# InternRobotics/InternNav

Measured on NVIDIA H100. Metric: InternVLA-N1 policy-steps/sec (batch RGB-D+text->action), higher is better.
Workload: dtype bf16

## Files before the change

### include/n1b200.h

```cpp
#ifndef N1B200_H_
#define N1B200_H_

#include <stddef.h>
#include <stdint.h>

#ifdef __cplusplus
extern "C" {
#endif

typedef struct n1_ctx* n1_handle;

enum {
  N1_OK = 0,
  N1_ERR_UNKNOWN = -1,
  N1_ERR_ARG = -2,
  N1_ERR_CUDA = -3,
  N1_ERR_NO_DEVICE = -4,
  N1_ERR_TMA = -5,
  N1_ERR_WEIGHT = -6,
  N1_ERR_WORKSPACE = -7
};

enum { N1_F32 = 0, N1_BF16 = 1 };

// ... 182 lines not shown
                int accumulate, void* ws, size_t ws_bytes, void* stream);
int n1_op_scale_cols(const void* x_bf16, int ld_x, const void* gamma_f32, const void* add_bf16_or_null, int ld_add,
                     void* out_bf16, int ld_out, int64_t rows, int cols, void* stream);
int n1_op_patchify_depth(const void* img_f32, void* out_bf16, int n_img, int ldk, void* stream);
int n1_op_adamw(void* master_f32, void* working_bf16_or_null, const void* grad_f32, void* m_f32, void* v_f32, int64_t n,
                float lr, float beta1, float beta2, float eps, float weight_decay, int step, void* stream);

void n1_prof_enable(int on);
void n1_prof_add(int64_t gemm_launches, int64_t total_launches);
int n1_prof_read(double* gemm_ms, double* gemm_flops, int64_t* gemm_launches, int64_t* total_launches);
int n1_prof_read_shapes(int32_t* mnk, int64_t* count, double* ms, int cap);

int n1_op_gemm(const void* A_bf16, int lda, const void* W_bf16, int ldw, void* out, int ldo, int M, int N, int K,
               const float* bias, const float* gamma, const void* residual_bf16, int ldr, int act, int out_fp32,
               void* stream);
int n1_op_ff_block(const void* x_bf16, int ldx, const float* ln_w, const float* ln_b, float eps, const void* w1_bf16,
                   const float* b1, const void* w2_bf16, const float* b2, void* out_bf16, int ldo, int M, void* stream);
int n1_op_dec_sa_block(void* x_bf16, int ldx, const float* ln_w, const float* ln_b, float eps, const void* w_qkv_bf16,
                       const float* b_qkv, const void* w_o_bf16, const float* b_o, int B, int Ns, int T, int causal,
                       void* stream);
int n1_op_dec_ca_block(void* x_bf16, int ldx, const float* ln_w, const float* ln_b, float eps, const void* w_q_bf16,
                       const float* b_q, const void* w_o_bf16, const float* b_o, const void* kv_bf16, int ldkv, int mtok,
                       int B, int Ns, int T, void* stream);
int n1_op_layernorm(const void* x_bf16, int ldx, void* y_bf16, int ldy, const float* w, const float* b, int rows, int D,
                    float eps, int rms, void* stream);
int n1_op_mod_norm(const void* x_bf16, int ldx, const float* w, const void* mod_bf16, int ld_mod, int rows_per_group,
                   const void* res_bf16, int ldr, void* out_bf16, int ldo, int64_t rows, int D, float eps, int mode,
                   void* stream);
int n1_op_add(const void* a_bf16, const void* b_bf16, void* out_bf16, int64_t n, void* stream);
int n1_op_action_embed(const float* lat, const float* w, const float* b, const float* pos, void* out_bf16, int64_t rows,
                       int T, int D, void* stream);
int n1_op_cfg_euler(const void* pred_bf16, int ld, int64_t n, int cfg, float scale, float dt, float* lat, void* stream);
int n1_op_attention(const void* q, const void* k, const void* v, void* o, int ldq, int ldk, int ldv, int ldo, int heads_q,
                    int heads_kv, int head_dim, int batch, int seq_q, int seq_k, const int32_t* cu_q,
                    const int32_t* cu_k, int max_seq_q, int kv_div, int causal, float scale, void* stream);

int n1_op_attention_ex(const void* q, const void* k, const void* v, void* o, int ldq, int ldk, int ldv, int ldo, int heads_q,
                       int heads_kv, int head_dim, int batch, const int32_t* cu_seqlens, int max_seq, int64_t total_rows,
                       int causal, float scale, int* used_tcgen05, void* stream);

int n1_op_attention_cache(const void* q, int ldq, int64_t q_rows, const void* k, const void* v, int ldkv, int64_t kv_rows,
                          void* o, int ldo, const int32_t* cu_q, const int32_t* ctx, const int32_t* row0, int batch,
                          int max_chunk, int heads_q, int heads_kv, float scale, void* stream);

#ifdef __cplusplus
}
// ... 3 lines not shown
```

### internnav_b200/_lib.py

```python
import ctypes
import os
import threading

import torch

_HERE = os.path.dirname(os.path.abspath(__file__))
LIB_PATH = os.path.join(_HERE, "libn1b200.so")

_lib = None
_lock = threading.Lock()

c_void_p, c_int, c_size_t, c_float, c_char_p = (
    ctypes.c_void_p, ctypes.c_int, ctypes.c_size_t, ctypes.c_float, ctypes.c_char_p)


class N1Error(RuntimeError):
    def __init__(self, code, msg):
        super().__init__("n1b200 error %d: %s" % (code, msg))
        self.code = code


class TensorDesc(ctypes.Structure):
    _fields_ = [("name", c_char_p), ("data", c_void_p), ("dtype", ctypes.c_int32), ("ndim", ctypes.c_int32),
                ("shape", ctypes.c_int64 * 4)]
# ... 18 lines not shown
    "n1_navdp_eps": (c_int, [c_void_p, c_void_p, c_size_t, c_void_p, c_void_p, c_int, c_void_p, c_void_p, c_void_p,
                             c_int, c_int, c_int, c_void_p]),
    "n1_navdp_sample": (c_int, [c_void_p, c_void_p, c_size_t, c_void_p, c_void_p, c_void_p, c_void_p, c_void_p,
                                c_int, c_int, c_int, c_int, c_void_p]),
    "n1_ddpm_tables": (c_int, [c_int, ctypes.POINTER(c_float)]),
    "n1_rgb_tokens_workspace_bytes": (c_size_t, [c_void_p, c_int]),
    "n1_rgb_tokens": (c_int, [c_void_p, c_void_p, c_size_t, c_void_p, c_void_p, c_int, c_void_p]),
    "n1_traj_to_actions": (c_int, [c_void_p, c_int, c_int, c_int, ctypes.c_double, ctypes.c_double, c_int, c_int, c_int,
                                   c_void_p, c_void_p, c_void_p, c_void_p]),
    "n1_prof_enable": (None, [c_int]),
    "n1_prof_add": (None, [ctypes.c_int64, ctypes.c_int64]),
    "n1_prof_read": (c_int, [ctypes.POINTER(ctypes.c_double), ctypes.POINTER(ctypes.c_double),
                             ctypes.POINTER(ctypes.c_int64), ctypes.POINTER(ctypes.c_int64)]),
    "n1_prof_read_shapes": (c_int, [ctypes.POINTER(ctypes.c_int32), ctypes.POINTER(ctypes.c_int64),
                                    ctypes.POINTER(ctypes.c_double), c_int]),
    "n1_op_gemm": (c_int, [c_void_p, c_int, c_void_p, c_int, c_void_p, c_int, c_int, c_int, c_int, c_void_p, c_void_p,
                           c_void_p, c_int, c_int, c_int, c_void_p]),
    "n1_op_ff_block": (c_int, [c_void_p, c_int, c_void_p, c_void_p, c_float, c_void_p, c_void_p, c_void_p, c_void_p, c_void_p,
                               c_int, c_int, c_void_p]),
    "n1_op_dec_sa_block": (c_int, [c_void_p, c_int, c_void_p, c_void_p, c_float, c_void_p, c_void_p, c_void_p, c_void_p,
                                   c_int, c_int, c_int, c_int, c_void_p]),
    "n1_op_dec_ca_block": (c_int, [c_void_p, c_int, c_void_p, c_void_p, c_float, c_void_p, c_void_p, c_void_p, c_void_p,
                                   c_void_p, c_int, c_int, c_int, c_int, c_int, c_void_p]),
    "n1_op_layernorm": (c_int, [c_void_p, c_int, c_void_p, c_int, c_void_p, c_void_p, c_int, c_int, c_float, c_int,
                                c_void_p]),
    "n1_op_mod_norm": (c_int, [c_void_p, c_int, c_void_p, c_void_p, c_int, c_int, c_void_p, c_int, c_void_p, c_int,
                               ctypes.c_int64, c_int, c_float, c_int, c_void_p]),
    "n1_op_add": (c_int, [c_void_p, c_void_p, c_void_p, ctypes.c_int64, c_void_p]),
    "n1_op_action_embed": (c_int, [c_void_p, c_void_p, c_void_p, c_void_p, c_void_p, ctypes.c_int64, c_int, c_int, c_void_p]),
    "n1_op_cfg_euler": (c_int, [c_void_p, c_int, ctypes.c_int64, c_int, c_float, c_float, c_void_p, c_void_p]),
    "n1_op_attention_ex": (c_int, [c_void_p, c_void_p, c_void_p, c_void_p, c_int, c_int, c_int, c_int, c_int, c_int, c_int,
                                   c_int, c_void_p, c_int, ctypes.c_int64, c_int, c_float, ctypes.POINTER(c_int), c_void_p]),
    "n1_op_attention": (c_int, [c_void_p, c_void_p, c_void_p, c_void_p, c_int, c_int, c_int, c_int, c_int, c_int, c_int,
                                c_int, c_int, c_int, c_void_p, c_void_p, c_int, c_int, c_int, c_float, c_void_p]),
    "n1_op_attention_cache": (c_int, [c_void_p, c_int, ctypes.c_int64, c_void_p, c_void_p, c_int, ctypes.c_int64, c_void_p,
                                      c_int, c_void_p, c_void_p, c_void_p, c_int, c_int, c_int, c_int, c_float, c_void_p]),
}

OP_RGBD, OP_GOAL, OP_DENOISE = 1, 2, 3
ACT_NONE, ACT_GELU, ACT_RELU, ACT_SWIGLU, ACT_GELU_TANH, ACT_SILU = 0, 1, 2, 3, 4, 5


def lib():
    global _lib
    with _lock:
        if _lib is None:
# ... 155 lines not shown
    if scale is None:
        scale = head_dim ** -0.5
    used = c_int(0)
    check(lib().n1_op_attention_ex(c_void_p(q.data_ptr()), c_void_p(k.data_ptr()), c_void_p(v.data_ptr()), ptr(o),
                                   q.stride(0), k.stride(0), v.stride(0), o.stride(0), heads_q, heads_kv, head_dim,
                                   cu_seqlens.numel() - 1, ptr(cu_seqlens), int(max_seq), q.shape[0], 1 if causal else 0,
                                   float(scale), ctypes.byref(used), stream_ptr()))
    return o, bool(used.value)


def attention_cache(q, k, v, heads_q, heads_kv, cu_q, ctx, row0, max_chunk, scale=None, out=None):
    assert q.dtype == k.dtype == v.dtype == torch.bfloat16 and q.stride(1) == 1 and k.stride(1) == 1 and v.stride(1) == 1
    assert k.stride(0) == v.stride(0) and k.shape[0] == v.shape[0]
    for t in (cu_q, ctx, row0):
        assert t.dtype == torch.int32 and t.is_cuda and t.is_contiguous()
    o = torch.empty(q.shape[0], heads_q * 128, device=q.device, dtype=torch.bfloat16) if out is None else out
    check(lib().n1_op_attention_cache(c_void_p(q.data_ptr()), q.stride(0), q.shape[0], c_void_p(k.data_ptr()),
                                      c_void_p(v.data_ptr()), k.stride(0), k.shape[0], ptr(o), o.stride(0), ptr(cu_q),
                                      ptr(ctx), ptr(row0), cu_q.numel() - 1, int(max_chunk), heads_q, heads_kv,
                                      float(128 ** -0.5 if scale is None else scale), stream_ptr()))
    return o


def ff_block(x, ln_w, ln_b, w1, b1, w2, b2, eps=1e-5, out=None):
    assert x.dtype == torch.bfloat16 and x.shape[1] == 384 and w1.shape == (1536, 384) and w2.shape == (384, 1536)
    assert w1.is_contiguous() and w2.is_contiguous() and x.stride(1) == 1
    if out is None:
        out = torch.empty(x.shape[0], 384, device=x.device, dtype=torch.bfloat16)
    check(lib().n1_op_ff_block(c_void_p(x.data_ptr()), x.stride(0), ptr(ln_w), ptr(ln_b), eps, ptr(w1), ptr(b1), ptr(w2),
                               ptr(b2), c_void_p(out.data_ptr()), out.stride(0), x.shape[0], stream_ptr()))
    return out


def dec_sa_block(x, ln_w, ln_b, w_qkv, b_qkv, w_o, b_o, B, Ns, T, causal=True, eps=1e-5):
    assert x.dtype == torch.bfloat16 and x.shape == (B * Ns * T, 384) and x.stride(1) == 1
    assert w_qkv.shape == (1152, 384) and w_o.shape == (384, 384)
    check(lib().n1_op_dec_sa_block(c_void_p(x.data_ptr()), x.stride(0), ptr(ln_w), ptr(ln_b), float(eps), ptr(w_qkv),
                                   ptr(b_qkv), ptr(w_o), ptr(b_o), B, Ns, T, 1 if causal else 0, stream_ptr()))
    return x


def dec_ca_block(x, ln_w, ln_b, w_q, b_q, w_o, b_o, kv, mtok, B, Ns, T, eps=1e-5):
    assert x.dtype == torch.bfloat16 and x.shape == (B * Ns * T, 384) and x.stride(1) == 1
    assert w_q.shape == (384, 384) and w_o.shape == (384, 384) and kv.shape[0] == B * mtok and kv.stride(1) == 1
    check(lib().n1_op_dec_ca_block(c_void_p(x.data_ptr()), x.stride(0), ptr(ln_w), ptr(ln_b), float(eps), ptr(w_q), ptr(b_q),
                                   ptr(w_o), ptr(b_o), c_void_p(kv.data_ptr()), kv.stride(0), mtok, B, Ns, T, stream_ptr()))
    return x
```

### internnav_b200/csrc/api.cu

```cuda
#include <string.h>

#include <string>
#include <vector>

#include "../../include/n1b200.h"
#include "n1_ops.h"
#include "resize.h"
#include "bwd_kernels.h"
#include "s1_model.h"
#include "s2_kernels.h"
#include "s2_model.h"
#include "weights.h"

using namespace n1;

struct n1_ctx {
  int device = 0;
  S1Model s1;
  S2Model s2;
};
struct n1_vit_plan_s {
  VitPlan* p;
};
struct n1_llm_plan_s {
// ... 735 lines not shown
    e.bias = bias, e.gamma = gamma, e.residual = B16(residual), e.ldr = ldr, e.act = act, e.out_fp32 = out_fp32;
    gemm_bf16(B16(A), lda, B16(W), ldw, out, ldo, M, N, K, e, S(stream));
  });
}

int n1_test_gemm(const void* A, int lda, const void* W, int ldw, void* out, int ldo, int M, int N, int K, const float* bias,
                 const float* gamma, const void* residual, int ldr, int act, int out_fp32, int rows_per_group,
                 int group_stride, int group_offset, const float* row_add, int tile_n, void* stream) {
  return guard([&] {
    GemmEpilogue e;
    e.bias = bias, e.gamma = gamma, e.residual = B16(residual), e.ldr = ldr, e.act = act, e.out_fp32 = out_fp32;
    e.rows_per_group = rows_per_group, e.group_stride = group_stride, e.group_offset = group_offset, e.row_add = row_add;
    gemm_bf16(B16(A), lda, B16(W), ldw, out, ldo, M, N, K, e, S(stream), tile_n);
  });
}

int n1_op_ff_block(const void* x, int ldx, const float* ln_w, const float* ln_b, float eps, const void* w1, const float* b1,
                   const void* w2, const float* b2, void* out, int ldo, int M, void* stream) {
  return guard([&] {
    ff_block_384(B16(x), ldx, ln_w, ln_b, eps, B16(w1), b1, B16(w2), b2, B16(out), ldo, M, S(stream));
  });
}

int n1_op_dec_sa_block(void* x, int ldx, const float* ln_w, const float* ln_b, float eps, const void* w_qkv,
                       const float* b_qkv, const void* w_o, const float* b_o, int B, int Ns, int T, int causal, void* stream) {
  return guard([&] {
    dec_sa_block(B16(x), ldx, ln_w, ln_b, eps, B16(w_qkv), b_qkv, B16(w_o), b_o, B, Ns, T, causal, S(stream));
  });
}
int n1_op_dec_ca_block(void* x, int ldx, const float* ln_w, const float* ln_b, float eps, const void* w_q, const float* b_q,
                       const void* w_o, const float* b_o, const void* kv, int ldkv, int mtok, int B, int Ns, int T,
                       void* stream) {
  return guard([&] {
    dec_ca_block(B16(x), ldx, ln_w, ln_b, eps, B16(w_q), b_q, B16(w_o), b_o, B16(kv), ldkv, mtok, B, Ns, T, S(stream));
  });
}

int n1_op_mod_norm(const void* x, int ldx, const float* w, const void* mod, int ld_mod, int rows_per_group, const void* res,
                   int ldr, void* out, int ldo, int64_t rows, int D, float eps, int mode, void* stream) {
  return guard([&] {
    mod_norm(B16(x), ldx, w, B16(mod), ld_mod, rows_per_group, B16(res), ldr, B16(out), ldo, rows, D, eps, mode, S(stream));
  });
}
int n1_op_add(const void* a, const void* b, void* out, int64_t n, void* stream) {
  return guard([&] { add_bf16(B16(a), B16(b), B16(out), n, S(stream)); });
}
// ... 56 lines not shown
```

### internnav_b200/csrc/dec_attn_block.cu

```cuda
#include <mutex>

#include "dec_tile.cuh"

namespace n1 {
namespace {

constexpr int D = 384, HD = 48, BM = 64;
constexpr int kABytes = BM * D * 2;
constexpr int kSlots = 2, kSlotBytes = D * 64 * 2;
constexpr int kKvRow = 112;
constexpr int kKvBytes = BM * kKvRow;
constexpr int kConsumerWarps = 8;
constexpr int kThreads = 32 * kConsumerWarps + 128;
constexpr int kSmem = 2 * kABytes + kSlots * kSlotBytes + 2 * 2 * kKvBytes + 256 + 1024;
static_assert(kSmem <= 232448, "dec_attn_block: shared memory budget (227 KB per block)");

struct DecAttnArgs {
  bf16* x;
  int ldx;
  const float* ln_w;
  const float* ln_b;
  float eps;
  const float* b_in;
  const float* b_o;
  const bf16* kv;
  int ldkv;
  int mtok;
  int Ns, T, tpt, tiles_per_env, tiles;
  int causal;
};

__device__ __forceinline__ void warpgroup_barrier(int g) { asm volatile("bar.sync %0, 128;" ::"r"(2 + g) : "memory"); }

template <bool kSelf>
__global__ void __launch_bounds__(kThreads, 1)
dec_attn_kernel(const __grid_constant__ CUtensorMap tmIn, const __grid_constant__ CUtensorMap tmO, const DecAttnArgs args) {
  constexpr int NP = kSelf ? 3 * HD : HD;
  constexpr int kHeadBytes = NP * 64 * 2;
  extern __shared__ uint8_t smem_raw[];
  uint8_t* smem = reinterpret_cast<uint8_t*>((reinterpret_cast<uintptr_t>(smem_raw) + 1023) & ~uintptr_t(1023));
  uint8_t* sA = smem;
  uint8_t* sO = smem + kABytes;
  uint8_t* sW = sO + kABytes;
  uint8_t* sKV = sW + kSlots * kSlotBytes;
  uint64_t* bars = reinterpret_cast<uint64_t*>(sKV + 4 * kKvBytes);
  uint64_t* full = bars;
  uint64_t* empty = bars + kSlots;

  const int warp = threadIdx.x >> 5, lane = threadIdx.x & 31;
  if (threadIdx.x == 0) {
    tma_prefetch_desc(&tmIn), tma_prefetch_desc(&tmO);
    for (int s = 0; s < kSlots; ++s) mbar_init(&full[s], 1), mbar_init(&empty[s], kConsumerWarps);
    fence_mbar_init();
  }
  __syncthreads();

  if (warp >= kConsumerWarps) {
    setmaxnreg_dec<kProducerRegs>();
    if (warp == kConsumerWarps && lane == 0) {
      Ring<kSlots> r;
      for (int t = blockIdx.x; t < args.tiles; t += gridDim.x) {
        for (int hp = 0; hp < 4; ++hp)
          for (int kb = 0; kb < D / 64; ++kb) {
            mbar_wait(&empty[r.slot], r.phase ^ 1);
            mbar_arrive_expect_tx(&full[r.slot], 2 * kHeadBytes);
            uint8_t* dst = sW + r.slot * kSlotBytes;
#pragma unroll
            for (int g = 0; g < 2; ++g) {
              const int h = 4 * g + hp;
#pragma unroll
              for (int part = 0; part < NP / HD; ++part)
                tma_load_2d(dst + g * kHeadBytes + part * HD * 128, &tmIn, &full[r.slot], kb * 64, part * D + h * HD);
            }
            r.advance();
          }
        for (int kb = 0; kb < D / 64; ++kb) {
          mbar_wait(&empty[r.slot], r.phase ^ 1);
          mbar_arrive_expect_tx(&full[r.slot], kSlotBytes);
          uint8_t* dst = sW + r.slot * kSlotBytes;
          tma_load_2d(dst, &tmO, &full[r.slot], kb * 64, 0);
          tma_load_2d(dst + kSlotBytes / 2, &tmO, &full[r.slot], kb * 64, 192);
          r.advance();
        }
      }
    }
  } else {
    setmaxnreg_inc<kConsumerRegs>();
    const int cw = warp;
    const int g = cw >> 2;
    const int wtid = threadIdx.x & 127;
    const int quad = lane & 3;
    const int r0 = (cw & 3) * 16 + (lane >> 2);
    uint8_t* sK = sKV + g * 2 * kKvBytes;
    uint8_t* sV = sK + kKvBytes;
    const float sl2 = 0.14433756729740643f * 1.4426950408889634f;
    Ring<kSlots> ring;
    for (int t = blockIdx.x; t < args.tiles; t += gridDim.x) {
      const int env = t / args.tiles_per_env;
      const int traj0 = (t - env * args.tiles_per_env) * args.tpt;
      const int ntraj = min(args.tpt, args.Ns - traj0);
      const long row0 = ((long)env * args.Ns + traj0) * args.T;
      const int nrows = ntraj * args.T;
      consumer_barrier();
      ln384_to_tile<false>(sA, args.x, args.ldx, row0, nrows, args.ln_w, args.ln_b, args.eps, cw, lane);
      fence_proxy_async_smem();
      consumer_barrier();
// ... 31 lines not shown
        int lo_key[2], hi_key[2];
#pragma unroll
        for (int r = 0; r < 2; ++r) {
          const int qi = r0 + 8 * r;
          if (kSelf) {
            lo_key[r] = qi / args.T * args.T;
            hi_key[r] = args.causal ? qi : lo_key[r] + args.T - 1;
          } else {
            lo_key[r] = 0, hi_key[r] = args.mtok - 1;
          }
        }
        float o[6][4], inv0, inv1;
        attn_hd48_16rows<4>(qf, sK, sV, kKvRow, lo_key, hi_key, sl2, lane, o, inv0, inv1);
#pragma unroll
        for (int i = 0; i < 6; ++i) {
          const int col = h * HD + i * 8 + quad * 2;
          *reinterpret_cast<uint32_t*>(sO + sw128_offset(r0, col)) = pack_bf16(o[i][0] * inv0, o[i][1] * inv0);
          *reinterpret_cast<uint32_t*>(sO + sw128_offset(r0 + 8, col)) = pack_bf16(o[i][2] * inv1, o[i][3] * inv1);
        }
      }
      fence_proxy_async_smem();
      consumer_barrier();
      float y[96] = {};
      mma_k384(y, sO, sW, full, empty, ring, kSlotBytes, g * (kSlotBytes / 2), lane, [] {});
      residual_epilogue_192<false>(y, args.x, args.ldx, args.x, args.ldx, args.b_o, row0, nrows, g, r0, quad);
    }
  }
}

template <bool kSelf>
void launch_dec_attn(const bf16* w_in, const bf16* w_o, const DecAttnArgs& a, long rows, cudaStream_t stream) {
  static std::once_flag once;
  std::call_once(once, [] { cudaFuncSetAttribute(dec_attn_kernel<kSelf>, cudaFuncAttributeMaxDynamicSharedMemorySize, kSmem); });
  const CUtensorMap tmIn = tma_map_2d(w_in, kSelf ? 3 * D : D, D, D, HD, 64, true);
  const CUtensorMap tmO = tma_map_2d(w_o, D, D, D, 192, 64, true);
  const int sms = device_sm_count();
  const int grid = a.tiles < sms ? a.tiles : sms;
  const int N = kSelf ? 4 * D : 2 * D;
  const double flops = 2.0 * rows * (double)N * D;
  const int ticket = prof_begin(flops, (int)rows, N, D, stream);
  dec_attn_kernel<kSelf><<<grid, kThreads, kSmem, stream>>>(tmIn, tmO, a);
  prof_end(ticket, stream);
  prof_count_gemm(flops);
  N1_CUDA(cudaGetLastError());
}

DecAttnArgs dec_args(bf16* x, int ldx, const float* ln_w, const float* ln_b, float eps, const float* b_in, const float* b_o,
                     int B, int Ns, int T) {
  N1_CHECK(x && ln_w && ln_b && b_in && b_o, "dec_attn_block: null pointer");
  N1_CHECK((reinterpret_cast<uintptr_t>(x) & 15) == 0 && ldx % 8 == 0 && ldx >= D, "dec_attn_block: misaligned x");
  N1_CHECK(B >= 1 && Ns >= 1 && T >= 1 && T <= BM, "dec_attn_block: needs B, Ns >= 1 and 1 <= T <= 64");
  DecAttnArgs a = {};
  a.x = x, a.ldx = ldx, a.ln_w = ln_w, a.ln_b = ln_b, a.eps = eps, a.b_in = b_in, a.b_o = b_o;
  a.Ns = Ns, a.T = T, a.tpt = BM / T;
  a.tiles_per_env = (Ns + a.tpt - 1) / a.tpt;
  const long tiles = (long)B * a.tiles_per_env;
  N1_CHECK(tiles < (1L << 31), "dec_attn_block: too many tiles");
  a.tiles = (int)tiles;
  return a;
}
// ... 24 lines not shown
```

### internnav_b200/csrc/dec_tile.cuh

```cuda
#pragma once
#include "n1_ops.h"
#include "n1_ptx.cuh"

namespace n1 {

__device__ __forceinline__ int sw128_offset(int row, int col) {
  return (col >> 6) * 8192 + (row >> 3) * 1024 + (row & 7) * 128 + ((((col & 63) >> 3) ^ (row & 7)) << 4) + (col & 7) * 2;
}

template <int kS>
struct Ring {
  int slot = 0;
  uint32_t phase = 0;
  __device__ __forceinline__ void advance() {
    if (++slot == kS) slot = 0, phase ^= 1;
  }
};

template <bool kNc>
__device__ __forceinline__ void ln384_to_tile(uint8_t* sA, const bf16* x, long ldx, long row0, int nrows, const float* ln_w,
                                              const float* ln_b, float eps, int cw, int lane) {
  constexpr int D = 384;
  uint2 q[8][3];
#pragma unroll
// ... 27 lines not shown
      const float c = bf16_lo(q[rr][i].y) - mu, d = bf16_hi(q[rr][i].y) - mu;
      sq[rr] += a * a + b * b + c * c + d * d;
    }
  }
#pragma unroll
  for (int o = 16; o > 0; o >>= 1)
#pragma unroll
    for (int rr = 0; rr < 8; ++rr) sq[rr] += __shfl_xor_sync(0xffffffffu, sq[rr], o);
#pragma unroll
  for (int i = 0; i < 3; ++i) {
    const int col = (lane + i * 32) * 4;
    const float4 lw = __ldg(reinterpret_cast<const float4*>(ln_w + col));
    const float4 lb = __ldg(reinterpret_cast<const float4*>(ln_b + col));
#pragma unroll
    for (int rr = 0; rr < 8; ++rr) {
      const float mu = s[rr], rstd = rsqrtf(sq[rr] * (1.0f / D) + eps);
      const float y0 = (bf16_lo(q[rr][i].x) - mu) * rstd * lw.x + lb.x, y1 = (bf16_hi(q[rr][i].x) - mu) * rstd * lw.y + lb.y;
      const float y2 = (bf16_lo(q[rr][i].y) - mu) * rstd * lw.z + lb.z, y3 = (bf16_hi(q[rr][i].y) - mu) * rstd * lw.w + lb.w;
      *reinterpret_cast<uint2*>(sA + sw128_offset(cw * 8 + rr, col)) = make_uint2(pack_bf16(y0, y1), pack_bf16(y2, y3));
    }
  }
}

template <int N, int kS, typename AfterFirst>
__device__ __forceinline__ void mma_k384(float (&acc)[N], const uint8_t* sA, const uint8_t* ring, uint64_t* full,
                                         uint64_t* empty, Ring<kS>& rs, int slot_bytes, int b_offset, int lane,
                                         AfterFirst after_first) {
  int prev = -1;
#pragma unroll 1
  for (int kb = 0; kb < 6; ++kb) {
    mbar_wait(&full[rs.slot], rs.phase);
    const uint64_t ad = wgmma_desc_sw128(smem_u32(sA + kb * 8192));
    const uint64_t bd = wgmma_desc_sw128(smem_u32(ring + rs.slot * slot_bytes + b_offset));
    wgmma_fence();
#pragma unroll
    for (int k = 0; k < 4; ++k) wgmma_ss<0, 0>(acc, ad + 2 * k, bd + 2 * k, (kb | k) != 0 ? 1u : 0u);
    wgmma_commit();
    wgmma_wait<1>();
    if (kb == 0) after_first();
    if (lane == 0 && prev >= 0) mbar_arrive(&empty[prev]);
    prev = rs.slot;
    rs.advance();
  }
  wgmma_wait<0>();
  if (lane == 0) mbar_arrive(&empty[prev]);
}

template <bool kNc>
__device__ __forceinline__ void residual_epilogue_192(const float (&y)[96], const bf16* x, long ldx, bf16* out, long ldo,
                                                      const float* bias, long row0, int nrows, int g, int r0, int quad) {
#pragma unroll
  for (int hh = 0; hh < 2; ++hh) {
    const int r = r0 + hh * 8;
    if (r >= nrows) continue;
    const bf16* xr = x + (row0 + r) * ldx + g * 192 + quad * 2;
    bf16* orow = out + (row0 + r) * ldo + g * 192 + quad * 2;
#pragma unroll
    for (int jj = 0; jj < 24; ++jj) {
      const uint32_t* xp = reinterpret_cast<const uint32_t*>(xr + jj * 8);
      const uint32_t xv = kNc ? __ldg(xp) : *xp;
      const float2 b = __ldg(reinterpret_cast<const float2*>(bias + g * 192 + jj * 8 + quad * 2));
      *reinterpret_cast<uint32_t*>(orow + jj * 8) =
          pack_bf16(y[jj * 4 + 2 * hh] + bf16_lo(xv) + b.x, y[jj * 4 + 2 * hh + 1] + bf16_hi(xv) + b.y);
    }
  }
}

template <int NKP>
// ... 64 lines not shown
```

### internnav_b200/csrc/ff_block.cu

```cuda
#include <mutex>

#include "dec_tile.cuh"

namespace n1 {
namespace {

constexpr int D = 384, F = 1536, BM = 64, HC = 128;
constexpr int NCH = F / HC;
constexpr int kS1 = 3, kS1Bytes = HC * 64 * 2;
constexpr int kS2 = 2, kS2Bytes = D * 64 * 2;
constexpr int kABytes = BM * D * 2;
constexpr int kHBytes = BM * HC * 2;
constexpr int kConsumerWarps = 8;
constexpr int kThreads = 32 * kConsumerWarps + 128;
constexpr int kSmem = kABytes + 2 * kHBytes + kS1 * kS1Bytes + kS2 * kS2Bytes + 256 + 1024;
static_assert(kSmem <= 232448, "ff_block: shared memory budget (227 KB per block)");

struct FfArgs {
  int M;
  int tiles_m;
  const bf16* x;
  int ldx;
  const float* ln_w;
  const float* ln_b;
  float eps;
  const float* b1;
  const float* b2;
  bf16* out;
  int ldo;
};

__global__ void __launch_bounds__(kThreads, 1)
ff_block_kernel(const __grid_constant__ CUtensorMap tmW1, const __grid_constant__ CUtensorMap tmW2, const FfArgs args) {
  extern __shared__ uint8_t smem_raw[];
  uint8_t* smem = reinterpret_cast<uint8_t*>((reinterpret_cast<uintptr_t>(smem_raw) + 1023) & ~uintptr_t(1023));
  uint8_t* sA = smem;
  uint8_t* sH = smem + kABytes;
  uint8_t* sW1 = sH + 2 * kHBytes;
  uint8_t* sW2 = sW1 + kS1 * kS1Bytes;
  uint64_t* bars = reinterpret_cast<uint64_t*>(sW2 + kS2 * kS2Bytes);
  uint64_t* w1_full = bars;
  uint64_t* w1_empty = bars + 3;
  uint64_t* w2_full = bars + 6;
  uint64_t* w2_empty = bars + 8;

  const int warp = threadIdx.x >> 5, lane = threadIdx.x & 31;
  if (threadIdx.x == 0) {
    tma_prefetch_desc(&tmW1), tma_prefetch_desc(&tmW2);
    for (int s = 0; s < kS1; ++s) mbar_init(&w1_full[s], 1), mbar_init(&w1_empty[s], kConsumerWarps);
    for (int s = 0; s < kS2; ++s) mbar_init(&w2_full[s], 1), mbar_init(&w2_empty[s], kConsumerWarps);
    fence_mbar_init();
  }
  __syncthreads();

  if (warp >= kConsumerWarps) {
    setmaxnreg_dec<kProducerRegs>();
    if (warp == kConsumerWarps && lane == 0) {
      Ring<kS1> r;
      for (int t = blockIdx.x; t < args.tiles_m; t += gridDim.x)
        for (int j = 0; j < NCH; ++j)
          for (int kb = 0; kb < D / 64; ++kb) {
            mbar_wait(&w1_empty[r.slot], r.phase ^ 1);
            mbar_arrive_expect_tx(&w1_full[r.slot], kS1Bytes);
            tma_load_2d(sW1 + r.slot * kS1Bytes, &tmW1, &w1_full[r.slot], kb * 64, j * HC);
            r.advance();
          }
    } else if (warp == kConsumerWarps + 1 && lane == 0) {
      Ring<kS2> r;
      for (int t = blockIdx.x; t < args.tiles_m; t += gridDim.x)
        for (int j = 0; j < NCH; ++j)
          for (int kb = 0; kb < HC / 64; ++kb) {
            mbar_wait(&w2_empty[r.slot], r.phase ^ 1);
            mbar_arrive_expect_tx(&w2_full[r.slot], kS2Bytes);
            uint8_t* dst = sW2 + r.slot * kS2Bytes;
            tma_load_2d(dst, &tmW2, &w2_full[r.slot], j * HC + kb * 64, 0);
            tma_load_2d(dst + kS2Bytes / 2, &tmW2, &w2_full[r.slot], j * HC + kb * 64, 192);
            r.advance();
          }
    }
  } else {
    setmaxnreg_inc<kConsumerRegs>();
    const int cw = warp;
    const int g = cw >> 2;
    const int quad = lane & 3;
    const int r0 = (cw & 3) * 16 + (lane >> 2);
    Ring<kS1> r1;
    Ring<kS2> r2;
    for (int tm = blockIdx.x; tm < args.tiles_m; tm += gridDim.x) {
      const long row0 = (long)tm * BM;
      consumer_barrier();
      ln384_to_tile<true>(sA, args.x, args.ldx, row0, args.M - tm * BM, args.ln_w, args.ln_b, args.eps, cw, lane);
      fence_proxy_async_smem();
      consumer_barrier();

      float y[96] = {};
      for (int j = 0; j < NCH; ++j) {
        float h[32];
        mma_k384(h, sA, sW1, w1_full, w1_empty, r1, kS1Bytes, g * 8192, lane, [&] {
          if (lane == 0 && j > 0) {
            mbar_arrive(&w2_empty[r2.slot]);
            mbar_arrive(&w2_empty[r2.slot ^ 1]);
          }
        });
        uint8_t* hb = sH + (j & 1) * kHBytes;
#pragma unroll
        for (int jj = 0; jj < 8; jj += 2) {
          float v[8];
#pragma unroll
          for (int u = 0; u < 2; ++u) {
            const float2 b = __ldg(reinterpret_cast<const float2*>(args.b1 + j * HC + g * 64 + (jj + u) * 8 + quad * 2));
            v[4 * u + 0] = h[(jj + u) * 4 + 0] + b.x, v[4 * u + 1] = h[(jj + u) * 4 + 1] + b.y;
            v[4 * u + 2] = h[(jj + u) * 4 + 2] + b.x, v[4 * u + 3] = h[(jj + u) * 4 + 3] + b.y;
          }
          gelu_erf8(v);
#pragma unroll
          for (int u = 0; u < 2; ++u)
#pragma unroll
            for (int hh = 0; hh < 2; ++hh)
              *reinterpret_cast<uint32_t*>(hb + sw128_offset(r0 + hh * 8, g * 64 + (jj + u) * 8 + quad * 2)) =
                  pack_bf16(v[4 * u + 2 * hh], v[4 * u + 2 * hh + 1]);
        }
        fence_proxy_async_smem();
        consumer_barrier();
        wgmma_fence();
#pragma unroll
        for (int kb = 0; kb < HC / 64; ++kb) {
          mbar_wait(&w2_full[r2.slot], r2.phase);
          const uint64_t ad = wgmma_desc_sw128(smem_u32(hb + kb * 8192));
          const uint64_t bd = wgmma_desc_sw128(smem_u32(sW2 + r2.slot * kS2Bytes + g * (kS2Bytes / 2)));
#pragma unroll
          for (int k = 0; k < 4; ++k) wgmma_ss<0, 0>(y, ad + 2 * k, bd + 2 * k, (j | kb | k) != 0 ? 1u : 0u);
          r2.advance();
        }
        wgmma_commit();
      }
      wgmma_wait<0>();
      if (lane == 0) {
        mbar_arrive(&w2_empty[r2.slot]);
        mbar_arrive(&w2_empty[r2.slot ^ 1]);
      }
      residual_epilogue_192<true>(y, args.x, args.ldx, args.out, args.ldo, args.b2, row0, args.M - tm * BM, g, r0, quad);
    }
  }
}

void launch_ff(const bf16* w1, const bf16* w2, const FfArgs& a, cudaStream_t stream) {
  static std::once_flag once;
  std::call_once(once, [] { cudaFuncSetAttribute(ff_block_kernel, cudaFuncAttributeMaxDynamicSharedMemorySize, kSmem); });
  const CUtensorMap tmW1 = tma_map_2d(w1, F, D, D, HC, 64, true);
  const CUtensorMap tmW2 = tma_map_2d(w2, D, F, F, 192, 64, true);
  const int sms = device_sm_count();
  const int grid = a.tiles_m < sms ? a.tiles_m : sms;
  const int ticket = prof_begin(4.0 * a.M * (double)D * F, a.M, -F, D, stream);
  ff_block_kernel<<<grid, kThreads, kSmem, stream>>>(tmW1, tmW2, a);
  prof_end(ticket, stream);
  prof_count_gemm(4.0 * a.M * (double)D * F);
  N1_CUDA(cudaGetLastError());
}

}

void ff_block_384(const bf16* x, int ldx, const float* ln_w, const float* ln_b, float eps, const bf16* w1, const float* b1,
                  const bf16* w2, const float* b2, bf16* out, int ldo, int M, cudaStream_t stream) {
  if (M <= 0) return;
  N1_CHECK(x && out && w1 && w2 && ln_w && ln_b && b1 && b2, "ff_block_384: null pointer");
  N1_CHECK((reinterpret_cast<uintptr_t>(x) & 15) == 0 && ldx % 8 == 0, "ff_block_384: misaligned x");
  N1_CHECK((reinterpret_cast<uintptr_t>(out) & 3) == 0 && ldo % 2 == 0, "ff_block_384: misaligned out");
  FfArgs a;
  a.M = M, a.tiles_m = (M + BM - 1) / BM;
  a.x = x, a.ldx = ldx, a.ln_w = ln_w, a.ln_b = ln_b, a.eps = eps, a.b1 = b1, a.b2 = b2, a.out = out, a.ldo = ldo;
  launch_ff(w1, w2, a, stream);
}

}
```

### internnav_b200/csrc/n1_ops.h

```cpp
#pragma once
#include <cuda.h>
#include <cuda_bf16.h>
#include <cuda_runtime.h>
#include <stdint.h>

#include <stdexcept>
#include <string>

namespace n1 {

typedef __nv_bfloat16 bf16;

struct Error : std::runtime_error {
  int code;
  Error(int c, const std::string& m) : std::runtime_error(m), code(c) {}
};

#define N1_CHECK(cond, msg)                                                                       \
  do {                                                                                            \
    if (!(cond)) throw ::n1::Error(-2, std::string(__FILE__) + ":" + std::to_string(__LINE__) + \
                                           ": " + (msg));                                         \
  } while (0)

#define N1_CUDA(call)                                                                              \
// ... 62 lines not shown
};
void attention(const AttnParams& p, cudaStream_t stream);
bool attention_tc_supported(const AttnParams& p);
bool attention_uses_tc(const AttnParams& p);
void attention_tc128(const AttnParams& p, cudaStream_t stream);

struct CacheAttnParams {
  const bf16* q;
  int ldq;
  long q_rows;
  const bf16 *k, *v;
  int ldkv;
  long kv_rows;
  bf16* o;
  int ldo;
  const int *cu_q, *ctx, *row0;
  int batch, max_chunk, heads_q, heads_kv;
  float scale;
};
void attention_cache(const CacheAttnParams& p, cudaStream_t stream);

void ff_block_384(const bf16* x, int ldx, const float* ln_w, const float* ln_b, float eps, const bf16* w1, const float* b1,
                  const bf16* w2, const float* b2, bf16* out, int ldo, int M, cudaStream_t stream);
void dec_sa_block(bf16* x, int ldx, const float* ln_w, const float* ln_b, float eps, const bf16* w_qkv, const float* b_qkv,
                  const bf16* w_o, const float* b_o, int B, int Ns, int T, int causal, cudaStream_t stream);
void dec_ca_block(bf16* x, int ldx, const float* ln_w, const float* ln_b, float eps, const bf16* w_q, const float* b_q,
                  const bf16* w_o, const float* b_o, const bf16* kv, int ldkv, int mtok, int B, int Ns, int T,
                  cudaStream_t stream);

void mod_norm(const bf16* x, int ldx, const float* w, const bf16* mod, int ld_mod, int rows_per_group, const bf16* res, int ldr,
              bf16* out, int ldo, long rows, int D, float eps, int mode, cudaStream_t stream);
void add_bf16(const bf16* a, const bf16* b, bf16* out, long n, cudaStream_t stream);
void action_embed(const float* lat, const float* w, const float* b, const float* pos, bf16* out, long rows, int T, int D,
                  cudaStream_t stream);
void cfg_euler(const bf16* pred, int ld, long n, int cfg, float scale, float dt, float* lat, cudaStream_t stream);

void traj_to_actions(const float* traj, int B, int Ns, int T, double turn_rad, double step_size, int lookahead,
                     int max_actions, int cap, int* ids, int* count, double* mean_out, cudaStream_t s);

}
```

Before: 66.54.

## Unify fused-block weight rings into finer-grained shared slots

The FF block kernel merges its separate W1 and W2 TMA rings (3 and 2 slots, two producer threads) into one 9-slot ring of 16 KB slots fed by a single producer. W2 k-blocks now span three consecutive slots. The cross-attention decoder kernel splits its weight ring into 8 smaller slots so W_o blocks span several slots, and mma_k384 gains a slots-per-k-block parameter. The aim is deeper prefetch and less stalling on weight loads, at the cost of more mbarrier waits and arrives per k-step. An optional grid-size cap knob is also added for experiments; it is off by default.

```diff
diff --git a/include/n1b200.h b/include/n1b200.h
--- a/include/n1b200.h
+++ b/include/n1b200.h
@@ -228,6 +228,7 @@
 int n1_op_dec_ca_block(void* x_bf16, int ldx, const float* ln_w, const float* ln_b, float eps, const void* w_q_bf16,
                        const float* b_q, const void* w_o_bf16, const float* b_o, const void* kv_bf16, int ldkv, int mtok,
                        int B, int Ns, int T, void* stream);
+int n1_op_dec_grid_cap(int ctas);
 int n1_op_layernorm(const void* x_bf16, int ldx, void* y_bf16, int ldy, const float* w, const float* b, int rows, int D,
                     float eps, int rms, void* stream);
 int n1_op_mod_norm(const void* x_bf16, int ldx, const float* w, const void* mod_bf16, int ld_mod, int rows_per_group,
diff --git a/internnav_b200/_lib.py b/internnav_b200/_lib.py
--- a/internnav_b200/_lib.py
+++ b/internnav_b200/_lib.py
@@ -64,6 +64,7 @@
                                    c_int, c_int, c_int, c_int, c_void_p]),
     "n1_op_dec_ca_block": (c_int, [c_void_p, c_int, c_void_p, c_void_p, c_float, c_void_p, c_void_p, c_void_p, c_void_p,
                                    c_void_p, c_int, c_int, c_int, c_int, c_int, c_void_p]),
+    "n1_op_dec_grid_cap": (c_int, [c_int]),
     "n1_op_layernorm": (c_int, [c_void_p, c_int, c_void_p, c_int, c_void_p, c_void_p, c_int, c_int, c_float, c_int,
                                 c_void_p]),
     "n1_op_mod_norm": (c_int, [c_void_p, c_int, c_void_p, c_void_p, c_int, c_int, c_void_p, c_int, c_void_p, c_int,
@@ -265,27 +266,40 @@
     return o
 
 
-def ff_block(x, ln_w, ln_b, w1, b1, w2, b2, eps=1e-5, out=None):
+def _grid_capped(max_ctas, launch):
+    if max_ctas is None:
+        return launch()
+    check(lib().n1_op_dec_grid_cap(int(max_ctas)))
+    try:
+        return launch()
+    finally:
+        check(lib().n1_op_dec_grid_cap(0))
+
+
+def ff_block(x, ln_w, ln_b, w1, b1, w2, b2, eps=1e-5, out=None, max_ctas=None):
     assert x.dtype == torch.bfloat16 and x.shape[1] == 384 and w1.shape == (1536, 384) and w2.shape == (384, 1536)
     assert w1.is_contiguous() and w2.is_contiguous() and x.stride(1) == 1
     if out is None:
         out = torch.empty(x.shape[0], 384, device=x.device, dtype=torch.bfloat16)
-    check(lib().n1_op_ff_block(c_void_p(x.data_ptr()), x.stride(0), ptr(ln_w), ptr(ln_b), eps, ptr(w1), ptr(b1), ptr(w2),
-                               ptr(b2), c_void_p(out.data_ptr()), out.stride(0), x.shape[0], stream_ptr()))
-    return out
-
-
-def dec_sa_block(x, ln_w, ln_b, w_qkv, b_qkv, w_o, b_o, B, Ns, T, causal=True, eps=1e-5):
+    _grid_capped(max_ctas, lambda: check(lib().n1_op_ff_block(
+        c_void_p(x.data_ptr()), x.stride(0), ptr(ln_w), ptr(ln_b), eps, ptr(w1), ptr(b1), ptr(w2), ptr(b2),
+        c_void_p(out.data_ptr()), out.stride(0), x.shape[0], stream_ptr())))
+    return out
+
+
+def dec_sa_block(x, ln_w, ln_b, w_qkv, b_qkv, w_o, b_o, B, Ns, T, causal=True, eps=1e-5, max_ctas=None):
     assert x.dtype == torch.bfloat16 and x.shape == (B * Ns * T, 384) and x.stride(1) == 1
     assert w_qkv.shape == (1152, 384) and w_o.shape == (384, 384)
-    check(lib().n1_op_dec_sa_block(c_void_p(x.data_ptr()), x.stride(0), ptr(ln_w), ptr(ln_b), float(eps), ptr(w_qkv),
-                                   ptr(b_qkv), ptr(w_o), ptr(b_o), B, Ns, T, 1 if causal else 0, stream_ptr()))
+    _grid_capped(max_ctas, lambda: check(lib().n1_op_dec_sa_block(
+        c_void_p(x.data_ptr()), x.stride(0), ptr(ln_w), ptr(ln_b), float(eps), ptr(w_qkv), ptr(b_qkv), ptr(w_o), ptr(b_o),
+        B, Ns, T, 1 if causal else 0, stream_ptr())))
     return x
 
 
-def dec_ca_block(x, ln_w, ln_b, w_q, b_q, w_o, b_o, kv, mtok, B, Ns, T, eps=1e-5):
+def dec_ca_block(x, ln_w, ln_b, w_q, b_q, w_o, b_o, kv, mtok, B, Ns, T, eps=1e-5, max_ctas=None):
     assert x.dtype == torch.bfloat16 and x.shape == (B * Ns * T, 384) and x.stride(1) == 1
     assert w_q.shape == (384, 384) and w_o.shape == (384, 384) and kv.shape[0] == B * mtok and kv.stride(1) == 1
-    check(lib().n1_op_dec_ca_block(c_void_p(x.data_ptr()), x.stride(0), ptr(ln_w), ptr(ln_b), float(eps), ptr(w_q), ptr(b_q),
-                                   ptr(w_o), ptr(b_o), c_void_p(kv.data_ptr()), kv.stride(0), mtok, B, Ns, T, stream_ptr()))
+    _grid_capped(max_ctas, lambda: check(lib().n1_op_dec_ca_block(
+        c_void_p(x.data_ptr()), x.stride(0), ptr(ln_w), ptr(ln_b), float(eps), ptr(w_q), ptr(b_q), ptr(w_o), ptr(b_o),
+        c_void_p(kv.data_ptr()), kv.stride(0), mtok, B, Ns, T, stream_ptr())))
     return x
diff --git a/internnav_b200/csrc/api.cu b/internnav_b200/csrc/api.cu
--- a/internnav_b200/csrc/api.cu
+++ b/internnav_b200/csrc/api.cu
@@ -781,6 +781,13 @@
   });
 }
 
+int n1_op_dec_grid_cap(int ctas) {
+  return guard([&] {
+    N1_CHECK(ctas >= 0, "n1_op_dec_grid_cap: needs ctas >= 0");
+    dec_grid_cap = ctas;
+  });
+}
+
 int n1_op_dec_sa_block(void* x, int ldx, const float* ln_w, const float* ln_b, float eps, const void* w_qkv,
                        const float* b_qkv, const void* w_o, const float* b_o, int B, int Ns, int T, int causal, void* stream) {
   return guard([&] {
diff --git a/internnav_b200/csrc/dec_attn_block.cu b/internnav_b200/csrc/dec_attn_block.cu
--- a/internnav_b200/csrc/dec_attn_block.cu
+++ b/internnav_b200/csrc/dec_attn_block.cu
@@ -7,12 +7,19 @@
 
 constexpr int D = 384, HD = 48, BM = 64;
 constexpr int kABytes = BM * D * 2;
-constexpr int kSlots = 2, kSlotBytes = D * 64 * 2;
+template <bool kSelf>
+struct WeightRing {
+  static constexpr int slots = kSelf ? 2 : 8;
+  static constexpr int bytes = 2 * D * 64 * 2 / slots;
+  static constexpr int wo_slots = D * 64 * 2 / bytes;
+  static_assert(slots % wo_slots == 0 && (4 * 6) % wo_slots == 0, "dec_attn_block: a W_o k-block must not wrap");
+};
+constexpr int kRingBytes = 2 * D * 64 * 2;
 constexpr int kKvRow = 112;
 constexpr int kKvBytes = BM * kKvRow;
 constexpr int kConsumerWarps = 8;
 constexpr int kThreads = 32 * kConsumerWarps + 128;
-constexpr int kSmem = 2 * kABytes + kSlots * kSlotBytes + 2 * 2 * kKvBytes + 256 + 1024;
+constexpr int kSmem = 2 * kABytes + kRingBytes + 2 * 2 * kKvBytes + 256 + 1024;
 static_assert(kSmem <= 232448, "dec_attn_block: shared memory budget (227 KB per block)");
 
 struct DecAttnArgs {
@@ -37,12 +44,15 @@
 dec_attn_kernel(const __grid_constant__ CUtensorMap tmIn, const __grid_constant__ CUtensorMap tmO, const DecAttnArgs args) {
   constexpr int NP = kSelf ? 3 * HD : HD;
   constexpr int kHeadBytes = NP * 64 * 2;
+  constexpr int kSlots = WeightRing<kSelf>::slots, kSlotBytes = WeightRing<kSelf>::bytes;
+  constexpr int kWoSlots = WeightRing<kSelf>::wo_slots;
+  static_assert(2 * kHeadBytes <= kSlotBytes, "dec_attn_block: an input-projection k-block fills one slot");
   extern __shared__ uint8_t smem_raw[];
   uint8_t* smem = reinterpret_cast<uint8_t*>((reinterpret_cast<uintptr_t>(smem_raw) + 1023) & ~uintptr_t(1023));
   uint8_t* sA = smem;
   uint8_t* sO = smem + kABytes;
   uint8_t* sW = sO + kABytes;
-  uint8_t* sKV = sW + kSlots * kSlotBytes;
+  uint8_t* sKV = sW + kRingBytes;
   uint64_t* bars = reinterpret_cast<uint64_t*>(sKV + 4 * kKvBytes);
   uint64_t* full = bars;
   uint64_t* empty = bars + kSlots;
@@ -74,14 +84,16 @@
             }
             r.advance();
           }
-        for (int kb = 0; kb < D / 64; ++kb) {
-          mbar_wait(&empty[r.slot], r.phase ^ 1);
-          mbar_arrive_expect_tx(&full[r.slot], kSlotBytes);
-          uint8_t* dst = sW + r.slot * kSlotBytes;
-          tma_load_2d(dst, &tmO, &full[r.slot], kb * 64, 0);
-          tma_load_2d(dst + kSlotBytes / 2, &tmO, &full[r.slot], kb * 64, 192);
-          r.advance();
-        }
+        for (int kb = 0; kb < D / 64; ++kb)
+          for (int i = 0; i < kWoSlots; ++i) {
+            mbar_wait(&empty[r.slot], r.phase ^ 1);
+            mbar_arrive_expect_tx(&full[r.slot], kSlotBytes);
+            uint8_t* dst = sW + r.slot * kSlotBytes;
+            const int box = D / (2 * kWoSlots);
+            tma_load_2d(dst, &tmO, &full[r.slot], kb * 64, (2 * i) * box);
+            tma_load_2d(dst + kSlotBytes / 2, &tmO, &full[r.slot], kb * 64, (2 * i + 1) * box);
+            r.advance();
+          }
       }
     }
   } else {
@@ -159,7 +171,7 @@
       fence_proxy_async_smem();
       consumer_barrier();
       float y[96] = {};
-      mma_k384(y, sO, sW, full, empty, ring, kSlotBytes, g * (kSlotBytes / 2), lane, [] {});
+      mma_k384<kWoSlots>(y, sO, sW, full, empty, ring, kSlotBytes, g * (D / 2 * 128), lane, [] {});
       residual_epilogue_192<false>(y, args.x, args.ldx, args.x, args.ldx, args.b_o, row0, nrows, g, r0, quad);
     }
   }
@@ -170,9 +182,10 @@
   static std::once_flag once;
   std::call_once(once, [] { cudaFuncSetAttribute(dec_attn_kernel<kSelf>, cudaFuncAttributeMaxDynamicSharedMemorySize, kSmem); });
   const CUtensorMap tmIn = tma_map_2d(w_in, kSelf ? 3 * D : D, D, D, HD, 64, true);
-  const CUtensorMap tmO = tma_map_2d(w_o, D, D, D, 192, 64, true);
+  const CUtensorMap tmO = tma_map_2d(w_o, D, D, D, D / (2 * WeightRing<kSelf>::wo_slots), 64, true);
   const int sms = device_sm_count();
-  const int grid = a.tiles < sms ? a.tiles : sms;
+  int grid = a.tiles < sms ? a.tiles : sms;
+  if (dec_grid_cap > 0 && grid > dec_grid_cap) grid = dec_grid_cap;
   const int N = kSelf ? 4 * D : 2 * D;
   const double flops = 2.0 * rows * (double)N * D;
   const int ticket = prof_begin(flops, (int)rows, N, D, stream);
diff --git a/internnav_b200/csrc/dec_tile.cuh b/internnav_b200/csrc/dec_tile.cuh
--- a/internnav_b200/csrc/dec_tile.cuh
+++ b/internnav_b200/csrc/dec_tile.cuh
@@ -73,28 +73,33 @@
   }
 }
 
-template <int N, int kS, typename AfterFirst>
+template <int SPK = 1, int N, int kS, typename AfterFirst>
 __device__ __forceinline__ void mma_k384(float (&acc)[N], const uint8_t* sA, const uint8_t* ring, uint64_t* full,
                                          uint64_t* empty, Ring<kS>& rs, int slot_bytes, int b_offset, int lane,
                                          AfterFirst after_first) {
   int prev = -1;
 #pragma unroll 1
   for (int kb = 0; kb < 6; ++kb) {
-    mbar_wait(&full[rs.slot], rs.phase);
+    const int s0 = rs.slot;
+#pragma unroll
+    for (int i = 0; i < SPK; ++i) mbar_wait(&full[rs.slot], rs.phase), rs.advance();
     const uint64_t ad = wgmma_desc_sw128(smem_u32(sA + kb * 8192));
-    const uint64_t bd = wgmma_desc_sw128(smem_u32(ring + rs.slot * slot_bytes + b_offset));
+    const uint64_t bd = wgmma_desc_sw128(smem_u32(ring + s0 * slot_bytes + b_offset));
     wgmma_fence();
 #pragma unroll
     for (int k = 0; k < 4; ++k) wgmma_ss<0, 0>(acc, ad + 2 * k, bd + 2 * k, (kb | k) != 0 ? 1u : 0u);
     wgmma_commit();
     wgmma_wait<1>();
     if (kb == 0) after_first();
-    if (lane == 0 && prev >= 0) mbar_arrive(&empty[prev]);
-    prev = rs.slot;
-    rs.advance();
+    if (lane == 0 && prev >= 0)
+#pragma unroll
+      for (int i = 0; i < SPK; ++i) mbar_arrive(&empty[prev + i]);
+    prev = s0;
   }
   wgmma_wait<0>();
-  if (lane == 0) mbar_arrive(&empty[prev]);
+  if (lane == 0)
+#pragma unroll
+    for (int i = 0; i < SPK; ++i) mbar_arrive(&empty[prev + i]);
 }
 
 template <bool kNc>
diff --git a/internnav_b200/csrc/ff_block.cu b/internnav_b200/csrc/ff_block.cu
--- a/internnav_b200/csrc/ff_block.cu
+++ b/internnav_b200/csrc/ff_block.cu
@@ -7,14 +7,14 @@
 
 constexpr int D = 384, F = 1536, BM = 64, HC = 128;
 constexpr int NCH = F / HC;
-constexpr int kS1 = 3, kS1Bytes = HC * 64 * 2;
-constexpr int kS2 = 2, kS2Bytes = D * 64 * 2;
+constexpr int kSlots = 9, kSlotBytes = HC * 64 * 2;
 constexpr int kABytes = BM * D * 2;
 constexpr int kHBytes = BM * HC * 2;
 constexpr int kConsumerWarps = 8;
 constexpr int kThreads = 32 * kConsumerWarps + 128;
-constexpr int kSmem = kABytes + 2 * kHBytes + kS1 * kS1Bytes + kS2 * kS2Bytes + 256 + 1024;
+constexpr int kSmem = kABytes + 2 * kHBytes + kSlots * kSlotBytes + 256 + 1024;
 static_assert(kSmem <= 232448, "ff_block: shared memory budget (227 KB per block)");
+static_assert((D / 64) % 3 == 0 && kSlots % 3 == 0, "ff_block: a W2 k-block must not wrap around the ring");
 
 struct FfArgs {
   int M;
@@ -36,19 +36,15 @@
   uint8_t* smem = reinterpret_cast<uint8_t*>((reinterpret_cast<uintptr_t>(smem_raw) + 1023) & ~uintptr_t(1023));
   uint8_t* sA = smem;
   uint8_t* sH = smem + kABytes;
-  uint8_t* sW1 = sH + 2 * kHBytes;
-  uint8_t* sW2 = sW1 + kS1 * kS1Bytes;
-  uint64_t* bars = reinterpret_cast<uint64_t*>(sW2 + kS2 * kS2Bytes);
-  uint64_t* w1_full = bars;
-  uint64_t* w1_empty = bars + 3;
-  uint64_t* w2_full = bars + 6;
-  uint64_t* w2_empty = bars + 8;
+  uint8_t* sW = sH + 2 * kHBytes;
+  uint64_t* bars = reinterpret_cast<uint64_t*>(sW + kSlots * kSlotBytes);
+  uint64_t* full = bars;
+  uint64_t* empty = bars + kSlots;
 
   const int warp = threadIdx.x >> 5, lane = threadIdx.x & 31;
   if (threadIdx.x == 0) {
     tma_prefetch_desc(&tmW1), tma_prefetch_desc(&tmW2);
-    for (int s = 0; s < kS1; ++s) mbar_init(&w1_full[s], 1), mbar_init(&w1_empty[s], kConsumerWarps);
-    for (int s = 0; s < kS2; ++s) mbar_init(&w2_full[s], 1), mbar_init(&w2_empty[s], kConsumerWarps);
+    for (int s = 0; s < kSlots; ++s) mbar_init(&full[s], 1), mbar_init(&empty[s], kConsumerWarps);
     fence_mbar_init();
   }
   __syncthreads();
@@ -56,27 +52,19 @@
   if (warp >= kConsumerWarps) {
     setmaxnreg_dec<kProducerRegs>();
     if (warp == kConsumerWarps && lane == 0) {
-      Ring<kS1> r;
+      Ring<kSlots> r;
+      auto load = [&](const CUtensorMap* tm, int c0, int c1) {
+        mbar_wait(&empty[r.slot], r.phase ^ 1);
+        mbar_arrive_expect_tx(&full[r.slot], kSlotBytes);
+        tma_load_2d(sW + r.slot * kSlotBytes, tm, &full[r.slot], c0, c1);
+        r.advance();
+      };
       for (int t = blockIdx.x; t < args.tiles_m; t += gridDim.x)
-        for (int j = 0; j < NCH; ++j)
-          for (int kb = 0; kb < D / 64; ++kb) {
-            mbar_wait(&w1_empty[r.slot], r.phase ^ 1);
-            mbar_arrive_expect_tx(&w1_full[r.slot], kS1Bytes);
-            tma_load_2d(sW1 + r.slot * kS1Bytes, &tmW1, &w1_full[r.slot], kb * 64, j * HC);
-            r.advance();
-          }
-    } else if (warp == kConsumerWarps + 1 && lane == 0) {
-      Ring<kS2> r;
-      for (int t = blockIdx.x; t < args.tiles_m; t += gridDim.x)
-        for (int j = 0; j < NCH; ++j)
-          for (int kb = 0; kb < HC / 64; ++kb) {
-            mbar_wait(&w2_empty[r.slot], r.phase ^ 1);
-            mbar_arrive_expect_tx(&w2_full[r.slot], kS2Bytes);
-            uint8_t* dst = sW2 + r.slot * kS2Bytes;
-            tma_load_2d(dst, &tmW2, &w2_full[r.slot], j * HC + kb * 64, 0);
-            tma_load_2d(dst + kS2Bytes / 2, &tmW2, &w2_full[r.slot], j * HC + kb * 64, 192);
-            r.advance();
-          }
+        for (int j = 0; j < NCH; ++j) {
+          for (int kb = 0; kb < D / 64; ++kb) load(&tmW1, kb * 64, j * HC);
+          for (int kb = 0; kb < HC / 64; ++kb)
+            for (int i = 0; i < 3; ++i) load(&tmW2, j * HC + kb * 64, i * 128);
+        }
     }
   } else {
     setmaxnreg_inc<kConsumerRegs>();
@@ -84,8 +72,7 @@
     const int g = cw >> 2;
     const int quad = lane & 3;
     const int r0 = (cw & 3) * 16 + (lane >> 2);
-    Ring<kS1> r1;
-    Ring<kS2> r2;
+    Ring<kSlots> ring;
     for (int tm = blockIdx.x; tm < args.tiles_m; tm += gridDim.x) {
       const long row0 = (long)tm * BM;
       consumer_barrier();
@@ -94,13 +81,12 @@
       consumer_barrier();
 
       float y[96] = {};
+      int s2 = 0;
       for (int j = 0; j < NCH; ++j) {
         float h[32];
-        mma_k384(h, sA, sW1, w1_full, w1_empty, r1, kS1Bytes, g * 8192, lane, [&] {
-          if (lane == 0 && j > 0) {
-            mbar_arrive(&w2_empty[r2.slot]);
-            mbar_arrive(&w2_empty[r2.slot ^ 1]);
-          }
+        mma_k384(h, sA, sW, full, empty, ring, kSlotBytes, g * 8192, lane, [&] {
+          if (lane == 0 && j > 0)
+            for (int i = 0; i < 6; ++i) mbar_arrive(&empty[s2 + i < kSlots ? s2 + i : s2 + i - kSlots]);
         });
         uint8_t* hb = sH + (j & 1) * kHBytes;
 #pragma unroll
@@ -122,23 +108,23 @@
         }
         fence_proxy_async_smem();
         consumer_barrier();
+        s2 = ring.slot;
         wgmma_fence();
 #pragma unroll
         for (int kb = 0; kb < HC / 64; ++kb) {
-          mbar_wait(&w2_full[r2.slot], r2.phase);
+          const int s = ring.slot;
+#pragma unroll
+          for (int i = 0; i < 3; ++i) mbar_wait(&full[ring.slot], ring.phase), ring.advance();
           const uint64_t ad = wgmma_desc_sw128(smem_u32(hb + kb * 8192));
-          const uint64_t bd = wgmma_desc_sw128(smem_u32(sW2 + r2.slot * kS2Bytes + g * (kS2Bytes / 2)));
+          const uint64_t bd = wgmma_desc_sw128(smem_u32(sW + s * kSlotBytes + g * (D / 2 * 128)));
 #pragma unroll
           for (int k = 0; k < 4; ++k) wgmma_ss<0, 0>(y, ad + 2 * k, bd + 2 * k, (j | kb | k) != 0 ? 1u : 0u);
-          r2.advance();
         }
         wgmma_commit();
       }
       wgmma_wait<0>();
-      if (lane == 0) {
-        mbar_arrive(&w2_empty[r2.slot]);
-        mbar_arrive(&w2_empty[r2.slot ^ 1]);
-      }
+      if (lane == 0)
+        for (int i = 0; i < 6; ++i) mbar_arrive(&empty[s2 + i < kSlots ? s2 + i : s2 + i - kSlots]);
       residual_epilogue_192<true>(y, args.x, args.ldx, args.out, args.ldo, args.b2, row0, args.M - tm * BM, g, r0, quad);
     }
   }
@@ -147,10 +133,11 @@
 void launch_ff(const bf16* w1, const bf16* w2, const FfArgs& a, cudaStream_t stream) {
   static std::once_flag once;
   std::call_once(once, [] { cudaFuncSetAttribute(ff_block_kernel, cudaFuncAttributeMaxDynamicSharedMemorySize, kSmem); });
-  const CUtensorMap tmW1 = tma_map_2d(w1, F, D, D, HC, 64, true);
-  const CUtensorMap tmW2 = tma_map_2d(w2, D, F, F, 192, 64, true);
+  const CUtensorMap tmW1 = tma_map_2d(w1, F, D, D, 128, 64, true);
+  const CUtensorMap tmW2 = tma_map_2d(w2, D, F, F, 128, 64, true);
   const int sms = device_sm_count();
-  const int grid = a.tiles_m < sms ? a.tiles_m : sms;
+  int grid = a.tiles_m < sms ? a.tiles_m : sms;
+  if (dec_grid_cap > 0 && grid > dec_grid_cap) grid = dec_grid_cap;
   const int ticket = prof_begin(4.0 * a.M * (double)D * F, a.M, -F, D, stream);
   ff_block_kernel<<<grid, kThreads, kSmem, stream>>>(tmW1, tmW2, a);
   prof_end(ticket, stream);
@@ -159,6 +146,8 @@
 }
 
 }
+
+int dec_grid_cap = 0;
 
 void ff_block_384(const bf16* x, int ldx, const float* ln_w, const float* ln_b, float eps, const bf16* w1, const float* b1,
                   const bf16* w2, const float* b2, bf16* out, int ldo, int M, cudaStream_t stream) {
diff --git a/internnav_b200/csrc/n1_ops.h b/internnav_b200/csrc/n1_ops.h
--- a/internnav_b200/csrc/n1_ops.h
+++ b/internnav_b200/csrc/n1_ops.h
@@ -108,6 +108,7 @@
 
 void ff_block_384(const bf16* x, int ldx, const float* ln_w, const float* ln_b, float eps, const bf16* w1, const float* b1,
                   const bf16* w2, const float* b2, bf16* out, int ldo, int M, cudaStream_t stream);
+extern int dec_grid_cap;
 void dec_sa_block(bf16* x, int ldx, const float* ln_w, const float* ln_b, float eps, const bf16* w_qkv, const float* b_qkv,
                   const bf16* w_o, const float* b_o, int B, int Ns, int T, int causal, cudaStream_t stream);
 void dec_ca_block(bf16* x, int ldx, const float* ln_w, const float* ln_b, float eps, const bf16* w_q, const float* b_q,
```

Result: faster. 68.01 (median of 6 runs) (+2.2%).
